# matvogel/P2P-Bridge

Hardware: AMD Instinct MI355X
Metric: denoised points/sec (8192-pt patches, T=30) (higher is better)
Workload: dtype f32; 1 GPU; PVDS_PUNet xyz-only, 8192-pt patches, T=30 bridge steps, batch 32 per GPU (BASELINE configs[1]); patches_per_gpu=32, points_per_patch=8192, bridge_steps=30, parallelism=patch-shard x1, process_group_world_size=1, hipgraph=True, weights=seeded random init (26.44 M params)

## Files before the change

### include/p2pb_hip.h

```cpp
#ifndef P2PB_HIP_H
#define P2PB_HIP_H

#include <stddef.h>

#ifdef __cplusplus
extern "C" {
#endif

#define P2PB_EINVAL (-22)

#define P2PB_ABI_VERSION 13

int p2pb_version(void);
const char *p2pb_target_arch(void);
int p2pb_set_split_terms(int terms);
int p2pb_set_split_terms_thread(int terms);
int p2pb_get_split_terms(void);
int p2pb_set_deterministic(int on);
int p2pb_get_deterministic(void);
int p2pb_debug_pointwise_form(int cin, int cout, int npos, unsigned long long *launches);

int p2pb_voxel_coords(int b, int n, int r, int normalize, float eps, const float *coords, float *norm,
                      int *vox, void *stream);

// ... 220 lines not shown
size_t p2pb_pointwise_minmax_floats(int b, int cout, int npos, int pool_u, int flags);
int p2pb_pointwise_conv_pool_forward(int b, int cin, int cout, int npos, const float *in, const void *wp,
                                     const float *bias, const float *bias_b, const float *in_scale,
                                     const float *in_shift, int in_swish, int flags, float *out, float *stats_part,
                                     int pool_u, float *minmax, double fin_count_per_channel, int fin_groups,
                                     const float *fin_gamma, const float *fin_beta, const float *fin_style, int fin_style_stride,
                                     float fin_eps, float *fin_scale, float *fin_shift, float *fin_chmean, void *stream);
int p2pb_pointwise_conv_pool_gather(int b, int cin, int cout, int n, int m, int u, const float *zt, const float *cxt,
                                    const int *idx, const void *wp_split, const float *bias, const float *in_scale,
                                    const float *in_shift, int in_swish, float *stats_part, float *minmax,
                                    double fin_count_per_channel, int fin_groups, const float *fin_gamma, const float *fin_beta,
                                    const float *fin_style, int fin_style_stride, float fin_eps, float *fin_scale,
                                    float *fin_shift, float *fin_chmean, void *stream);
int p2pb_linear_rows(int b, int cin, int cout, const float *x, long x_stride, const float *w, long w_stride,
                     const float *bias, float *out, long out_stride, void *stream);
int p2pb_minmax_act(int b, int c, int m, int nslots, const float *minmax, const float *scale, const float *shift,
                    int swish, float *y, void *stream);
int p2pb_minmax_act_pool_gn(int b, int c, int nslots, const float *minmax, const float *part, int nslots_st,
                            double count_per_channel, int groups, const float *gamma, const float *beta, const float *style,
                            int style_stride, float eps, int swish, float *scale, float *shift, float *y, void *stream);
int p2pb_affine_act(int b, int c, int npos, const float *x, const float *scale, const float *shift, int swish,
                    const float *residual, float *y, void *stream);
int p2pb_affine_act_max(int b, int c, int m, int u, const float *x, const float *scale, const float *shift,
                        int swish, float *y, void *stream);

int p2pb_linear_attention_forward(int b, int heads, int dim_head, int n, const float *qkv, float *out, float *ctx,
                                  void *stream);
int p2pb_linear_attention_backward(int b, int heads, int dim_head, int n, const float *qkv, const float *ctx,
                                   const float *grad_out, float *grad_qkv, void *stream);

// ... 154 lines not shown
```

### p2p_bridge_amd/_lib.py

```python
import ctypes
import os

import torch

_HERE = os.path.dirname(os.path.abspath(__file__))
LIB_PATH = os.environ.get("P2PB_LIB_PATH") or os.path.join(_HERE, "libp2pb_hip.so")

SYMBOLS = [
    "p2pb_version", "p2pb_target_arch", "p2pb_set_split_terms", "p2pb_set_split_terms_thread", "p2pb_get_split_terms", "p2pb_set_deterministic", "p2pb_get_deterministic", "p2pb_voxel_coords", "p2pb_avg_voxelize_ws_bytes",
    "p2pb_avg_voxelize_forward", "p2pb_avg_voxelize_backward", "p2pb_avg_voxelize_cl_gather_split", "p2pb_conv3d_presplit",
    "p2pb_conv3d_k3_forward_compact_pre", "p2pb_trilinear_devoxelize_forward",
    "p2pb_trilinear_devoxelize_backward", "p2pb_ball_query", "p2pb_grouping_forward", "p2pb_grouping_backward", "p2pb_group_concat", "p2pb_group_sub", "p2pb_three_interpolate_add", "p2pb_group_sub_stats_floats", "p2pb_group_sub_stats_slots", "p2pb_group_sub_stats",
    "p2pb_gather_features_forward", "p2pb_gather_features_backward", "p2pb_furthest_point_sampling",
    "p2pb_fps_coop_ws_bytes", "p2pb_furthest_point_sampling_coop", "p2pb_point_face_dist", "p2pb_face_point_dist", "p2pb_knn_points_ws_bytes", "p2pb_knn_points", "p2pb_three_nn_interpolate_forward", "p2pb_three_nn_interpolate_backward", "p2pb_three_nn", "p2pb_three_nn_cells", "p2pb_three_nn_cells_ws_bytes",
    "p2pb_three_interpolate", "p2pb_chamfer_forward",
    "p2pb_chamfer_backward", "p2pb_approxmatch_forward", "p2pb_matchcost_forward", "p2pb_matchcost_backward",
    "p2pb_auction_forward", "p2pb_auction_backward", "p2pb_conv3d_k3_packed_floats", "p2pb_conv3d_k3_pack_weights",
    "p2pb_conv3d_k3_split_packed_bytes", "p2pb_conv3d_k3_pack_weights_split",
    "p2pb_conv3d_k3_stats_floats", "p2pb_conv3d_k3_forward", "p2pb_conv3d_k3_forward_ex",
    "p2pb_conv3d_k3_far_field", "p2pb_conv3d_k3_far_field_gn", "p2pb_pvconv_tail", "p2pb_minmax_act_pool_gn", "p2pb_conv3d_active_lists", "p2pb_conv3d_k3_forward_compact", "p2pb_conv3d_brick_lists", "p2pb_conv3d_k3_forward_sparse", "p2pb_gn_affine_params", "p2pb_se_gate_affine",
    "p2pb_trilinear_devoxelize_affine", "p2pb_avg_voxelize_cl_forward", "p2pb_voxel_sort", "p2pb_avg_voxelize_cl_gather", "p2pb_trilinear_devoxelize_cl_affine", "p2pb_pointwise_packed_floats", "p2pb_pointwise_pack_weights",
    "p2pb_pointwise_stats_floats", "p2pb_pointwise_conv_forward", "p2pb_affine_act", "p2pb_affine_act_max",
    "p2pb_pointwise_split_packed_bytes", "p2pb_pointwise_pack_weights_split", "p2pb_pointwise_pool_supported", "p2pb_pointwise_minmax_floats", "p2pb_pointwise_conv_pool_forward",
    "p2pb_minmax_act", "p2pb_linear_attention_forward", "p2pb_linear_attention_backward", "p2pb_softmax_attention_forward", "p2pb_softmax_attention_backward",
    "p2pb_approxmatch_temp_floats", "p2pb_approxmatch_forward_ws", "p2pb_pointwise_conv_pool_gather", "p2pb_chamfer_ws_bytes", "p2pb_chamfer_forward_ws", "p2pb_radius_count", "p2pb_radius_fill", "p2pb_merge_accumulate", "p2pb_merge_finish", "p2pb_gn_affine_params_ex", "p2pb_norm_act_backward", "p2pb_norm_act_backward_ex", "p2pb_grouping_backward_pitched", "p2pb_three_nn_interpolate_backward_pitched", "p2pb_affine_act_train", "p2pb_conv3d_k3_wgrad_ws_floats", "p2pb_conv3d_k3_wgrad", "p2pb_conv3d_k3_wgrad_occ_ws_floats", "p2pb_conv3d_k3_wgrad_occ", "p2pb_pointwise_wgrad_ws_floats", "p2pb_pointwise_wgrad",
    "p2pb_debug_pointwise_form", "p2pb_linear_rows", "p2pb_fps_grid_ws_bytes", "p2pb_furthest_point_sampling_grid",
    "p2pb_optim_entry_bytes", "p2pb_optim_chunk", "p2pb_optim_clip_adam_step",
    "p2pb_conv3d_k3_pack_weights_split_adjoint", "p2pb_pointwise_pack_weights_adjoint", "p2pb_pointwise_pack_weights_split_adjoint",
    "p2pb_conv3d_k3_pack_weights_split_amax", "p2pb_pointwise_pack_weights_split_amax",
    "p2pb_se_gate_forward", "p2pb_se_gate_backward", "p2pb_row_max_forward", "p2pb_row_max_backward",
    "p2pb_pairwise_chamfer_ws_bytes", "p2pb_pairwise_chamfer", "p2pb_pairwise_emd_ws_bytes", "p2pb_pairwise_emd",
    "p2pb_occupancy_grid_cells", "p2pb_occupancy_ws_bytes", "p2pb_occupancy_counts",
    "p2pb_pn2_ball_query", "p2pb_pn2_three_nn", "p2pb_pn2_fps", "p2pb_pn2_three_interpolate", "p2pb_pn2_three_interpolate_grad",
    "p2pb_pointops_knnquery", "p2pb_pointops_ballquery", "p2pb_pointops_furthestsampling", "p2pb_pointops_grouping_forward",
    "p2pb_pointops_grouping_backward", "p2pb_pointops_interpolation_forward", "p2pb_pointops_interpolation_backward",
    "p2pb_pointops_subtraction_forward", "p2pb_pointops_subtraction_backward", "p2pb_pointops_aggregation_forward",
    "p2pb_pointops_aggregation_backward",
    "p2pb_imgfeat_visibility_ws_bytes", "p2pb_imgfeat_visibility", "p2pb_imgfeat_fuse", "p2pb_imgfeat_fill_round",
    "p2pb_scan_depth_valid", "p2pb_scan_backproject", "p2pb_scan_cell_keys", "p2pb_scan_segment_mean", "p2pb_scan_big_chunk_rows",
    "p2pb_scan_segment_mean_big", "p2pb_scan_radius_count", "p2pb_scan_knn_grid", "p2pb_scan_knn_brute",
    "p2pb_pairs_tri_areas", "p2pb_pairs_sample_mesh", "p2pb_pairs_knn", "p2pb_pairs_unique_assign", "p2pb_pairs_finish",
# ... 38 lines not shown
        _lib.p2pb_pointwise_minmax_floats.restype = ctypes.c_size_t
        _lib.p2pb_group_sub_stats_floats.restype = ctypes.c_size_t
        _lib.p2pb_pointwise_split_packed_bytes.restype = ctypes.c_size_t
        _lib.p2pb_conv3d_k3_wgrad_ws_floats.restype = ctypes.c_size_t
        _lib.p2pb_conv3d_k3_wgrad_occ_ws_floats.restype = ctypes.c_size_t
        _lib.p2pb_chamfer_ws_bytes.restype = ctypes.c_size_t
        _lib.p2pb_approxmatch_temp_floats.restype = ctypes.c_size_t
        _lib.p2pb_pointwise_wgrad_ws_floats.restype = ctypes.c_size_t
        _lib.p2pb_optim_entry_bytes.restype = ctypes.c_size_t
        _lib.p2pb_pairwise_chamfer_ws_bytes.restype = ctypes.c_size_t
        _lib.p2pb_pairwise_emd_ws_bytes.restype = ctypes.c_size_t
        _lib.p2pb_occupancy_ws_bytes.restype = ctypes.c_size_t
        _lib.p2pb_imgfeat_visibility_ws_bytes.restype = ctypes.c_size_t
        _lib.p2pb_vit_patch_embed_ws_floats.restype = ctypes.c_size_t
        _lib.p2pb_room_fps_jobs_ws_bytes.restype = ctypes.c_size_t
        have = _lib.p2pb_version() if hasattr(_lib, "p2pb_version") else None
        if have != ABI_VERSION:
            bad, _lib = _lib, None
            del bad
            raise P2PBError(f"{LIB_PATH} is ABI version {have}, this package binds version {ABI_VERSION} (include/p2pb_hip.h): "
                            "rebuild it with `python -m p2p_bridge_amd.build`")
        for s in SYMBOLS:
            getattr(_lib, s)
        _lib.p2pb_set_split_terms(6 if os.environ.get("P2PB_CONV_MATH") in ("bf16x6", "fp32") else 16)
    return _lib


def stream_ptr():
    return ctypes.c_void_p(torch.cuda.current_stream().cuda_stream)


# ... 18 lines not shown
```

### p2p_bridge_amd/csrc/pointwise_act.hip

```cpp
#include "pw_common.h"

__global__ __launch_bounds__(256) void minmax_act_kernel(int c, int m, int nslots, const float *__restrict__ mm,
                                                         const float *__restrict__ scale,
                                                         const float *__restrict__ shift, int swish,
                                                         float *__restrict__ y, size_t total) {
  for (size_t e = (size_t)blockIdx.x * 256 + threadIdx.x; e < total; e += (size_t)gridDim.x * 256) {
    float mn, mx;
    size_t bc;
    if (nslots == 0) {
      bc = e / m;
      const float2 v = *(const float2 *)(mm + e * 2);
      mn = v.x;
      mx = v.y;
    } else {
      bc = e;
      const size_t b = e / c, ch = e % c;
      mn = INFINITY;
      mx = -INFINITY;
      for (int sl = 0; sl < nslots; ++sl) {
        const float2 v = *(const float2 *)(mm + ((b * nslots + sl) * c + ch) * 2);
        mn = fminf(mn, v.x);
        mx = fmaxf(mx, v.y);
      }
    }
// ... 64 lines not shown
                                       double count_per_channel, int groups, const float *gamma, const float *beta,
                                       const float *style, int style_stride, float eps, int swish, float *scale, float *shift,
                                       float *y, void *stream) {
  if (b <= 0 || c <= 0 || nslots <= 0 || !minmax || !part || nslots_st <= 0 || !scale || !shift || !y || groups <= 0 ||
      c % groups != 0 || c / groups > 256 || (style && style_stride < 2 * c) || (size_t)c * 8 > 32 * 1024)
    return P2PB_EINVAL;
  GnFinish f = {};
  f.gamma = gamma, f.beta = beta, f.style = style, f.scale = scale, f.shift = shift, f.style_stride = style_stride, f.groups = groups;
  f.eps = eps, f.count_per_channel = count_per_channel;
  hipLaunchKernelGGL(minmax_act_pool_kernel, dim3((c + 31) / 32, b), dim3(256), (size_t)c * 8, (hipStream_t)stream, c, nslots, minmax,
                     (const float *)nullptr, (const float *)nullptr, swish, y, part, nslots_st, f);
  return p2pb_launch_status();
}

#define LR_BC 16
__global__ __launch_bounds__(256) void linear_rows_kernel(int B, int cin, int cout, const float *__restrict__ x, long xs,
                                                          const float *__restrict__ w, long ws,
                                                          const float *__restrict__ bias, float *__restrict__ out, long os,
                                                          int bc) {
  extern __shared__ float lr_x[];
  const int tid = threadIdx.x, lane = tid & 63, wave = tid >> 6, l31 = lane & 31, h = lane >> 5;
  const int row0 = blockIdx.x * 32;
  const int xp = cin + 4;
  const int wrow = min(row0 + l31, cout - 1);
  const int nk8 = (cin + 7) / 8;
  for (int b0 = 0; b0 < B; b0 += bc) {
    const int nb = min(bc, B - b0);
    __syncthreads();
    for (int e = tid * 4; e < nb * cin; e += 1024) {
      const int bb = e / cin, c = e - bb * cin;
      *(f32x4 *)(lr_x + bb * xp + c) = *(const f32x4 *)(x + (size_t)(b0 + bb) * xs + c);
    }
    __syncthreads();
    f32x16 acc;
// ... 20 lines not shown
      for (int u = 0; u < 8; ++u)
#pragma unroll
        for (int i = 0; i < 4; ++i) acc = __builtin_amdgcn_mfma_f32_32x32x2f32(wv[u][i], xv[u][i], acc, 0, 0, 0);
    }
    __syncthreads();
    float *red = lr_x;
    if (l31 < nb) {
#pragma unroll
      for (int r = 0; r < 16; ++r) red[(wave * 32 + (r & 3) + 8 * (r >> 2) + 4 * h) * 17 + l31] = acc[r];
    }
    __syncthreads();
    for (int e = tid; e < 32 * nb; e += 256) {
      const int r = e / nb, bb = e - r * nb;
      if (row0 + r < cout) {
        const float v = (red[(0 * 32 + r) * 17 + bb] + red[(1 * 32 + r) * 17 + bb]) + (red[(2 * 32 + r) * 17 + bb] + red[(3 * 32 + r) * 17 + bb]);
        out[(size_t)(b0 + bb) * os + row0 + r] = v + (bias ? bias[row0 + r] : 0.0f);
      }
    }
  }
}

extern "C" int p2pb_linear_rows(int b, int cin, int cout, const float *x, long x_stride, const float *w, long w_stride,
                                const float *bias, float *out, long out_stride, void *stream) {
  if (b <= 0 || cin <= 0 || cout <= 0 || !x || !w || !out || (cin & 3) || (x_stride & 3) || (w_stride & 3) ||
      (((uintptr_t)x | (uintptr_t)w) & 15) || x_stride < cin || w_stride < cin || out_stride < cout)
    return P2PB_EINVAL;
  int bc = (int)(65536 / ((long)(cin + 4) * 4));
  if (bc < 1) return P2PB_EINVAL;
  if (bc > LR_BC) bc = LR_BC;
  if (bc > b) bc = b;
  size_t lr_lds = (size_t)bc * (cin + 4) * 4;
  if (lr_lds < 4 * 32 * 17 * 4) lr_lds = 4 * 32 * 17 * 4;
  hipLaunchKernelGGL(linear_rows_kernel, dim3(cdiv(cout, 32)), dim3(256), lr_lds, (hipStream_t)stream, b, cin,
                     cout, x, x_stride, w, w_stride, bias, out, out_stride, bc);
  return p2pb_launch_status();
}

__global__ __launch_bounds__(256) void affine_act_kernel(int c, int P, const float *__restrict__ x,
                                                         const float *__restrict__ scale,
                                                         const float *__restrict__ shift, int swish,
                                                         const float *__restrict__ residual, float *__restrict__ y) {
  const int bc = blockIdx.y;
  const float sc = scale[bc], sh = shift[bc];
  const float *xr = x + (size_t)bc * P;
  const float *rr = residual ? residual + (size_t)bc * P : nullptr;
  float *yr = y + (size_t)bc * P;
  for (int p = blockIdx.x * 256 + threadIdx.x; p < P; p += gridDim.x * 256) {
    float v = xr[p] * sc + sh;
    if (swish) v = swishf(v);
// ... 98 lines not shown
```

### p2p_bridge_amd/fused.py

```python
import ctypes
import os

from . import _experiment
import threading

import torch

from ._lib import call, check, lib, ptr, stream_ptr

_i, _f, _d = ctypes.c_int, ctypes.c_float, ctypes.c_double
F32 = torch.float32


CONV_MATHS = ("f16x3", "bf16x6", "fp32")
SPLIT_MATHS = ("f16x3", "bf16x6")
CONV_MATH_DEFAULT = "f16x3"
_SPLIT_TERMS = {"f16x3": 16, "bf16x6": 6, "fp32": 6, "bf16x3": 3}
_conv_math_override = None


def conv_math() -> str:
    m = _conv_math_override or os.environ.get("P2PB_CONV_MATH", CONV_MATH_DEFAULT)
    if m not in CONV_MATHS:
        raise ValueError(f"P2PB_CONV_MATH must be one of {CONV_MATHS}, got {m!r}")
# ... 467 lines not shown

def linear_rows(x, weight, bias=None):
    if x.stride(-1) != 1 or x.data_ptr() % 16 or x.stride(0) % 4:
        x = x.contiguous()
    if weight.stride(-1) != 1 or weight.data_ptr() % 16 or weight.stride(0) % 4:
        weight = weight.contiguous()
    b, ci = x.shape
    co = weight.shape[0]
    assert weight.shape[1] == ci and x.dtype == F32 and weight.dtype == F32 and x.is_cuda
    out = torch.empty(b, co, dtype=F32, device=x.device)
    call("p2pb_linear_rows", _i(b), _i(ci), _i(co), ptr(x), ctypes.c_long(x.stride(0)), ptr(weight), ctypes.c_long(weight.stride(0)),
         ptr(bias), ptr(out), ctypes.c_long(co), stream_ptr())
    return out


def minmax_act(mm, scale, shift, swish=True, global_pool=False):
    if global_pool:
        b, nslots, c, _ = mm.shape
        y = torch.empty(b, c, dtype=F32, device=mm.device)
        m = 1
    else:
        b, c, m, _ = mm.shape
        nslots = 0
        y = torch.empty(b, c, m, dtype=F32, device=mm.device)
    call("p2pb_minmax_act", _i(b), _i(c), _i(m), _i(nslots), ptr(mm), ptr(scale), ptr(shift), _i(int(swish)), ptr(y),
         stream_ptr())
    return y


def gather_pool_supported(ci: int, co: int, m: int, u: int) -> bool:
# ... 132 lines not shown
```

### p2p_bridge_amd/p2pb.py

```python
import os
import warnings
from typing import Dict, List, Optional

import numpy as np
import torch
import torch.nn as nn

from .pvcnn_unet import PVCNN2Unet, _get


def space_indices(num_steps: int, count: int) -> List[int]:
    assert count <= num_steps
    stride = 1 if count <= 1 else (num_steps - 1) / (count - 1)
    cur, out = 0.0, []
    for _ in range(count):
        out.append(round(cur))
        cur += stride
    return out


def make_beta_schedule(n_timestep=1000, linear_start=1e-4, linear_end=2e-2):
    scale = 1000 / n_timestep
    a, b = (linear_start * scale) ** 0.5, (linear_end * scale) ** 0.5
    return (torch.linspace(a, b, n_timestep, dtype=torch.float64) ** 2).numpy()
# ... 232 lines not shown
        B = xt.shape[0]
        t = coef[0].expand(B)
        if self.cond_x1:
            x_cond = x1 if x_cond is None else torch.cat([x1, x_cond], dim=1)
        out = net(xt, t, x_cond=x_cond)
        if self.objective == "pred_noise":
            x0 = xt - coef[1] * out
            if clip:
                x0 = x0.clamp(-3.0, 3.0)
        else:
            x0 = out
        xt_prev = coef[2] * x0 + coef[3] * xt
        if noise is not None:
            xt_prev = xt_prev + coef[4] * noise
        return xt_prev, x0

    @torch.no_grad()
    def ddpm_sampling(self, x1, x_cond=None, clip_denoise=False, sampling_steps=None, log_count=10, verbose=True,
                      use_ema=False, graph=False):
        from . import fused

        args = (x1, x_cond, clip_denoise, sampling_steps, log_count, verbose, use_ema, graph)
        xs, x0s = self._ddpm_once(*args)
        policy = self.f16_overflow or os.environ.get("P2PB_F16_OVERFLOW", "rerun")
        if policy not in ("rerun", "raise", "ignore"):
            raise ValueError(f"P2PB_F16_OVERFLOW must be rerun | raise | ignore, got {policy!r}")
        if policy == "ignore" or fused.conv_math() != "f16x3" or xs.device.type != "cuda":
            return xs, x0s
        if bool(torch.isfinite(xs[:, 0]).all()):
            return xs, x0s
# ... 35 lines not shown
        if ema_was_training:
            self.ema.ema_model.eval()
        if self.add_x1_noise:
            x1 = x1 + torch.randn_like(x1)
        xt = x1.detach().to(self.device)
        xs, x0s = [], []
        rev = steps[::-1]
        chains = self._sampler_chains(xt) if graph else 1
        if chains > 1:
            try:
                return self._ddpm_chains(net, xt, x_cond, clip_denoise, rev, table, log_steps, chains)
            finally:
                if ema_was_training:
                    self.ema.ema_model.train()
                self.model.train()
        runner = self._graph_runner(net, xt, x_cond, clip_denoise) if graph else None
        try:
            for i, prev in enumerate(rev[1:]):
                noise = torch.randn_like(xt) if (not self.ot_ode and prev > 0) else None
                if runner is not None:
                    xt, x0 = runner(xt, table[i], noise)
                else:
                    xt, x0 = self._one_step(net, xt, table[i], x1, x_cond, clip_denoise, noise)
                if prev in log_steps:
                    xs.append(xt.clone() if runner is not None else xt)
                    x0s.append(x0.clone() if runner is not None else x0)
        finally:
            if ema_was_training:
                self.ema.ema_model.train()
            self.model.train()
        flip = lambda z: torch.flip(torch.stack(z, dim=1), dims=(1,))
        return flip(xs), flip(x0s)

    def _sampler_chains(self, xt) -> int:
        v = self.sample_chains if self.sample_chains is not None else os.environ.get("P2PB_SAMPLE_CHAINS")
        B, N = xt.shape[0], xt.shape[2]
        auto = 2 if (B % 2 == 0 and ((B >= 16 and N <= 16384) or (B >= 32 and N > 16384))) else 1
        k = int(v) if v not in (None, "", "auto") else auto
        return max(1, min(k, B))

    def _ddpm_chains(self, net, xt, x_cond, clip, rev, table, log_steps, chains):
        B = xt.shape[0]
        cuts = [(B * c) // chains for c in range(chains + 1)]
        parts = [slice(cuts[c], cuts[c + 1]) for c in range(chains)]
        main = torch.cuda.current_stream()
        runners = [self._graph_runner(net, xt[p], None if x_cond is None else x_cond[p], clip, chain=c)
                   for c, p in enumerate(parts)]
        streams = self._chain_streams = (getattr(self, "_chain_streams", None) or [])
        while len(streams) < chains:
            streams.append(torch.cuda.Stream(device=xt.device))
        if getattr(self, "_chains_serial", False):
            streams = [main] * chains
        x_c = [xt[p] for p in parts]
        logs = [([], []) for _ in parts]
        nsteps = len(rev) - 1
        for i, prev in enumerate(rev[1:]):
            noise = torch.randn_like(xt) if (not self.ot_ode and prev > 0) else None
            if noise is not None and i > 0:
                drawn = torch.cuda.Event()
                drawn.record(main)
                for c in range(chains):
                    streams[c].wait_event(drawn)
            if i == 0:
                from . import _experiment

                dflt = 0 if xt.shape[2] <= 16384 else 100
                phase = _experiment.get_int("chain_stagger_pct", dflt) / 100.0
                timed_first = phase > 0 and chains > 1 and nsteps > 1
                if timed_first:
                    e0, e1 = torch.cuda.Event(enable_timing=True), torch.cuda.Event(enable_timing=True)
                    e0.record(main)
                    x_c[0], x0 = runners[0](x_c[0], table[0], None if noise is None else noise[parts[0]])
                    e1.record(main)
                    if prev in log_steps:
                        logs[0][0].append(x_c[0].clone()), logs[0][1].append(x0.clone())
                    e1.synchronize()
                    step_ms = e0.elapsed_time(e1)
                for c in range(chains):
                    streams[c].wait_stream(main)
                    if timed_first and c > 0:
                        with torch.cuda.stream(streams[c]):
                            torch.cuda._sleep(int(step_ms * c / chains * phase * 1.8e6))
            for c in range(chains):
                if i == 0 and c == 0 and timed_first:
                    continue
                with torch.cuda.stream(streams[c]):
                    x_c[c], x0 = runners[c](x_c[c], table[i], None if noise is None else noise[parts[c]])
                    if prev in log_steps:
                        logs[c][0].append(x_c[c].clone()), logs[c][1].append(x0.clone())
                    if noise is not None:
                        noise.record_stream(streams[c])
        for c in range(chains):
            main.wait_stream(streams[c])
        flip = lambda z: torch.flip(torch.stack(z, dim=1), dims=(1,))
        xs = torch.cat([flip(l[0]) for l in logs], dim=0)
        x0s = torch.cat([flip(l[1]) for l in logs], dim=0)
        return xs, x0s

    @staticmethod
    def _weights_fingerprint(net):
        return tuple((t.data_ptr(), t._version) for t in list(net.parameters()) + list(net.buffers()))

    def _graph_runner(self, net, xt, x_cond, clip, chain=0):
        if self.cond_x1:
            raise NotImplementedError("graph capture with cond_x1")
        from . import fused

        key = (tuple(xt.shape), None if x_cond is None else tuple(x_cond.shape), bool(clip), id(net), fused.conv_math(), chain)
        fp = self._weights_fingerprint(net)
        entry = self._graphs.get(key)
        if entry is not None and entry[0] != fp:
            del self._graphs[key]
            entry = None
        if entry is None:
            s_x = xt.clone()
            s_c = torch.zeros(5, device=xt.device)
            s_n = None if self.ot_ode else torch.zeros_like(xt)
            s_cond = None if x_cond is None else x_cond.clone()
            self._one_step(net, s_x, s_c, None, s_cond, clip, s_n)
            torch.cuda.synchronize()
            side = torch.cuda.Stream()
            side.wait_stream(torch.cuda.current_stream())
            with torch.cuda.stream(side):
                for _ in range(2):
                    self._one_step(net, s_x, s_c, None, s_cond, clip, s_n)
            torch.cuda.current_stream().wait_stream(side)
            torch.cuda.synchronize()
            g = torch.cuda.CUDAGraph()
            with torch.cuda.graph(g, capture_error_mode="thread_local"):
                o_x, o_0 = self._one_step(net, s_x, s_c, None, s_cond, clip, s_n)
            entry = self._graphs[key] = (fp, g, s_x, s_c, s_n, s_cond, o_x, o_0)
        _, g, s_x, s_c, s_n, s_cond, o_x, o_0 = entry
        if s_cond is not None:
            s_cond.copy_(x_cond)

        def run(x, coef, noise=None):
            s_x.copy_(x)
            s_c.copy_(coef)
            if s_n is not None:
                if noise is None:
                    s_n.zero_()
                else:
                    s_n.copy_(noise)
            g.replay()
            return o_x, o_0

        return run

    @torch.no_grad()
    def calibrate_ranges(self, x_start, x_cond=None, steps=None, margin: float = 4.0, use_ema=False):
        from . import fused

        if fused.conv_math() != "f16x3" or self.device.type != "cuda":
            return []
        net = self.ema.ema_model if (use_ema and self.ema is not None) else self.model
        names = {id(m): n for n, m in net.named_modules()}
        was_training = net.training
        net.eval()
        _, table = self.step_tables(steps or self.timesteps - 1)
        xs = x_start.detach().to(self.device)
# ... 89 lines not shown
```

### p2p_bridge_amd/pvcnn_unet.py

```python
from dataclasses import dataclass
from typing import Any, List, Optional

import numpy as np
import os

import torch

from . import _experiment
import torch.nn as nn
import torch.nn.functional as F

from . import layers as L


def _get(cfg, key, default=None):
    if cfg is None:
        return default
    if isinstance(cfg, dict):
        v = cfg.get(key, None)
    else:
        v = getattr(cfg, key, None)
        if v is None and hasattr(cfg, "get"):
            v = cfg.get(key, None)
    return default if v is None else v


@dataclass
class PVCData:
    features: torch.Tensor
    coords: torch.Tensor = None
    cond_coords: torch.Tensor = None
    cond_features: torch.Tensor = None
    lower_coords: torch.Tensor = None
    lower_features: torch.Tensor = None
    time_emb: torch.Tensor = None
    cond: Any = None
    geo: Any = None
    lower_temb: torch.Tensor = None


def temb_broadcast(base, m):
    out = base[:, :, None].expand(-1, -1, m)
    out._p2pb_base = base
    return out


def temb_at(time_emb, m):
    base = getattr(time_emb, "_p2pb_base", None)
    if base is not None:
        return temb_broadcast(base, m)
    return time_emb[:, :, :m] if m <= time_emb.shape[-1] else time_emb[:, :, 0:1].expand(-1, -1, m)


# ... 602 lines not shown
        self.mlp = SharedMLP(in_channels, list(out_channels), dim=1, gn_groups=gn_groups, cond_dim=cond_dim)

    def forward(self, data: PVCData) -> PVCData:
        if data.geo is not None:
            idx, w = data.geo.take_fp(self.level)
            from . import fused

            if fused.enabled(self.mlp, data.lower_features):
                conv0 = self.mlp.layers[0]
                g = data.lower_features.contiguous()
                cg = g.shape[1]
                pm = g.shape[2] % 4 == 0
                tb = None
                if data.lower_temb is not None:
                    e = data.lower_temb.shape[1]
                    tb = fused.linear_rows(data.lower_temb, conv0.weight.reshape(conv0.weight.shape[0], -1)[:, cg:cg + e])
                cz, _ = fused.pw_conv(g, conv0, stats=False, ci_lo=0, ci_hi=cg, use_bias=False, point_major=pm, bias_b=tb)
                if tb is not None:
                    cg += data.lower_temb.shape[1]
                skip = data.features
                if skip is not None:
                    ys, _ = fused.pw_conv(skip.contiguous(), conv0, stats=False, ci_lo=cg, ci_hi=cg + skip.shape[1])
                    y, st = fused.interp_add(cz, idx, w, add=ys, point_major=pm)
                else:
                    y, st = fused.interp_add(cz, idx, w, bias=conv0.bias, point_major=pm)
                if data.time_emb is not None:
                    data.time_emb = data.time_emb[:, :, 0:1].expand(-1, -1, data.coords.shape[-1])
                data.features = self.mlp._run_fused(y, data.cond, False, None, first=st)
                return data
            x = L.three_interpolate(data.lower_features.contiguous(), idx, w)
        else:
# ... 121 lines not shown
        sa.append(dict(convs=convs, centers=ncen, radius=radius[i], neighbors=32, mlp_in=mlp_in, mlp_out=mlp_out))
        cin = mlp_out[-1]
    sa_in[0] = feat_dim + input_dim
    fp_mlps = [[channels[3], channels[3]], [channels[3], channels[3]], [channels[3], channels[2]],
               [channels[2], channels[2], channels[1]]]
    fp_conv = [(channels[3], n_fp_blocks[3], voxel_resolutions[3]), (channels[3], n_fp_blocks[2], voxel_resolutions[2]),
               (channels[2], n_fp_blocks[1], voxel_resolutions[1]), (channels[1], n_fp_blocks[0], voxel_resolutions[0])]
    fp = []
    for j in range(4):
        mlp_in = cin + sa_in[-1 - j] + embed_dim
        convs = []
        c = fp_mlps[j][-1]
        for _ in range(fp_conv[j][1]):
            convs.append(dict(cin=c, cout=fp_conv[j][0], r=int(fp_conv[j][2])))
            c = fp_conv[j][0]
        fp.append(dict(mlp_in=mlp_in, mlp_out=fp_mlps[j], convs=convs))
        cin = c
    return dict(sa=sa, fp=fp, bottleneck=sa[-1]["mlp_out"][-1], out=cin)


class Geometry:

    def __init__(self, plan, coords, side):
        main = torch.cuda.current_stream()
        self.main = main
        c0 = coords.contiguous()
        side.wait_stream(main)
        self.sa, self.fp = [], []
        from . import fused

        self.voxel = {}
# ... 162 lines not shown
        self._dec_adagn = None
        self._pass = {"drop_seed": None}
        for k, m in enumerate(m for m in self.modules() if isinstance(m, PVConv)):
            m._pass, m.drop_salt = self._pass, k + 1

    def get_timestep_embedding(self, timesteps, device=None):
        if timesteps.dim() == 2 and timesteps.shape[1] == 1:
            timesteps = timesteps[:, 0]
        assert timesteps.dim() == 1, f"get shape: {timesteps.shape}"
        e = timesteps[:, None] * self._temb_freq[None, :]
        e = torch.cat([torch.sin(e), torch.cos(e)], dim=1)
        if self.embed_dim % 2 == 1:
            e = F.pad(e, (0, 1), "constant", 0)
        return e

    def _decoder_adagns(self):
        if self._dec_adagn is None:
            self._dec_adagn = {id(m) for part in (self.global_att, self.fp_layers, self.classifier) if part is not None
                               for m in part.modules() if isinstance(m, AdaGN)}
        return self._dec_adagn

    def forward(self, x, t, x_cond=None):
        if x_cond is not None:
            x = torch.cat([x, x_cond], dim=1)
        B, C, N = x.shape
        assert C == self.input_dim + self.extra_feature_channels, \
            f"input dim: {C}, expected: {self.input_dim + self.extra_feature_channels}"
        coords = x[:, : self.input_dim].contiguous()
        feats = x[:, self.input_dim:].contiguous()
        from . import fused
# ... 29 lines not shown
            from . import dense

            if dense.fold_step_neighbours():
                self._pass["drop_seed"] = dense.dropout_seed(x.device)
        time_emb = None
        if t is not None:
            if t.dim() == 0:
                t = t.view(1).expand(B)
            te = self.get_timestep_embedding(t)
            if use_fused:
                te = fused.linear_rows(te, self.embedf[0].weight, self.embedf[0].bias)
                te = fused.linear_rows(F.leaky_relu(te, self.embedf[1].negative_slope), self.embedf[2].weight, self.embedf[2].bias)
            else:
                te = self.embedf(te)
            time_emb = temb_broadcast(te, N)
        data = PVCData(features=feats, coords=coords, time_emb=time_emb, cond=cond, geo=geo)

        skips, level_coords = [feats], []
        for i, stage in enumerate(self.sa_layers):
            if i > 0:
                skips.append(data.features)
            level_coords.append(data.coords)
            if i > 0 and data.time_emb is not None:
                data.features = torch.cat([data.features, data.time_emb], dim=1)
            data = stage(data)

        if self.collect_cut and torch.is_grad_enabled():
            def alias(x):
                return x.view_as(x) if x.requires_grad else x

# ... 8 lines not shown
                cut += cond.cut
            self.cut = [x for x in cut if x.requires_grad]

        if self.global_att is not None:
            data.features = self.global_att(data.features)

        for j, stage in enumerate(self.fp_layers):
            ltemb = None
            if data.time_emb is None:
                lower = data.features
            elif use_fused and geo is not None and data.time_emb.shape[1] % 4 == 0 and data.features.shape[1] % 4 == 0:
                lower, ltemb = data.features, data.time_emb[:, :, 0]
            else:
                lower = torch.cat([data.features, data.time_emb], dim=1)
            data = stage(PVCData(features=skips[-1 - j], coords=level_coords[-1 - j], lower_coords=data.coords,
                                 lower_features=lower, time_emb=data.time_emb, cond=data.cond, geo=geo, lower_temb=ltemb))
        if geo is not None:
            geo.finish()

        if use_fused:
            c0 = self.classifier[0]
            xin = data.features.contiguous()
            h, st, (sc, sh, _) = fused.pw_conv(xin, c0.layers[0], fin=norm_fin(c0.layers[1], xin.shape[2], None))
            return fused.pw_conv(h, self.classifier[2], sc, sh, swish=True, stats=False)[0]
        from . import dense

        seed = self._pass["drop_seed"]
        if seed is not None:
            h = self.classifier[0].run(data.features, None, dropout=(float(self.classifier[1].p), seed, 0))
        else:
            h = self.classifier[1](self.classifier[0].run(data.features, None))
# ... 2 lines not shown
```

Baseline: 1.230 million points/s.

## Fuse bridge update and step advance into captured graph; batch FP time biases

The per-step bridge update (x0 estimate, clamp, next xt with noise) becomes a single vectorized kernel captured inside the HIP graph. A device-side advance kernel reads the coefficient row from a table, so the host no longer copies coefficients or xt before each replay. The per-FP-stage time-embedding bias linears are also merged into one segmented linear launch at the start of the forward. Together these remove several small elementwise launches and host copies per step, at the cost of device-side step state that must be reset correctly for every sampling call.

```diff
diff --git a/include/p2pb_hip.h b/include/p2pb_hip.h
--- a/include/p2pb_hip.h
+++ b/include/p2pb_hip.h
@@ -258,6 +258,11 @@
                                     float *fin_shift, float *fin_chmean, void *stream);
 int p2pb_linear_rows(int b, int cin, int cout, const float *x, long x_stride, const float *w, long w_stride,
                      const float *bias, float *out, long out_stride, void *stream);
+int p2pb_linear_rows_segments(int b, int cin, int nseg, const int *seg_start, const float *x, long x_stride, const float *w,
+                              long w_stride, const float *bias, float *out, void *stream);
+int p2pb_bridge_step(long n, int pred_noise, int clamp, const float *xt, const float *out, const float *coef,
+                     const float *noise, float *x0, float *xt_prev, void *stream);
+int p2pb_bridge_advance(int reset, int nsteps, int cap, const float *table, int *state, float *coef, void *stream);
 int p2pb_minmax_act(int b, int c, int m, int nslots, const float *minmax, const float *scale, const float *shift,
                     int swish, float *y, void *stream);
 int p2pb_minmax_act_pool_gn(int b, int c, int nslots, const float *minmax, const float *part, int nslots_st,
diff --git a/p2p_bridge_amd/_lib.py b/p2p_bridge_amd/_lib.py
--- a/p2p_bridge_amd/_lib.py
+++ b/p2p_bridge_amd/_lib.py
@@ -24,7 +24,7 @@
     "p2pb_pointwise_split_packed_bytes", "p2pb_pointwise_pack_weights_split", "p2pb_pointwise_pool_supported", "p2pb_pointwise_minmax_floats", "p2pb_pointwise_conv_pool_forward",
     "p2pb_minmax_act", "p2pb_linear_attention_forward", "p2pb_linear_attention_backward", "p2pb_softmax_attention_forward", "p2pb_softmax_attention_backward",
     "p2pb_approxmatch_temp_floats", "p2pb_approxmatch_forward_ws", "p2pb_pointwise_conv_pool_gather", "p2pb_chamfer_ws_bytes", "p2pb_chamfer_forward_ws", "p2pb_radius_count", "p2pb_radius_fill", "p2pb_merge_accumulate", "p2pb_merge_finish", "p2pb_gn_affine_params_ex", "p2pb_norm_act_backward", "p2pb_norm_act_backward_ex", "p2pb_grouping_backward_pitched", "p2pb_three_nn_interpolate_backward_pitched", "p2pb_affine_act_train", "p2pb_conv3d_k3_wgrad_ws_floats", "p2pb_conv3d_k3_wgrad", "p2pb_conv3d_k3_wgrad_occ_ws_floats", "p2pb_conv3d_k3_wgrad_occ", "p2pb_pointwise_wgrad_ws_floats", "p2pb_pointwise_wgrad",
-    "p2pb_debug_pointwise_form", "p2pb_linear_rows", "p2pb_fps_grid_ws_bytes", "p2pb_furthest_point_sampling_grid",
+    "p2pb_debug_pointwise_form", "p2pb_linear_rows", "p2pb_bridge_step", "p2pb_bridge_advance", "p2pb_linear_rows_segments", "p2pb_fps_grid_ws_bytes", "p2pb_furthest_point_sampling_grid",
     "p2pb_optim_entry_bytes", "p2pb_optim_chunk", "p2pb_optim_clip_adam_step",
     "p2pb_conv3d_k3_pack_weights_split_adjoint", "p2pb_pointwise_pack_weights_adjoint", "p2pb_pointwise_pack_weights_split_adjoint",
     "p2pb_conv3d_k3_pack_weights_split_amax", "p2pb_pointwise_pack_weights_split_amax",
@@ -93,7 +93,7 @@
         _lib.p2pb_imgfeat_visibility_ws_bytes.restype = ctypes.c_size_t
         _lib.p2pb_vit_patch_embed_ws_floats.restype = ctypes.c_size_t
         _lib.p2pb_room_fps_jobs_ws_bytes.restype = ctypes.c_size_t
-        have = _lib.p2pb_version() if hasattr(_lib, "p2pb_version") else None
+        have =_lib.p2pb_version() if hasattr(_lib, "p2pb_version") else None
         if have != ABI_VERSION:
             bad, _lib = _lib, None
             del bad
diff --git a/p2p_bridge_amd/csrc/bridge_step.hip b/p2p_bridge_amd/csrc/bridge_step.hip
--- /dev/null
+++ b/p2p_bridge_amd/csrc/bridge_step.hip
@@ -0,0 +1,100 @@
+#include "common.h"
+
+typedef float bs_f4 __attribute__((ext_vector_type(4)));
+
+template <bool PRED_NOISE, bool CLAMP, bool NOISE>
+__device__ __forceinline__ void bridge_one(float xt, float out, float nz, float c1, float c2, float c3, float c4, float &x0,
+                                           float &xp) {
+  float v = out;
+  if (PRED_NOISE) {
+    v = __fsub_rn(xt, __fmul_rn(c1, out));
+    if (CLAMP) v = (v != v) ? v : fminf(fmaxf(v, -3.0f), 3.0f);
+  }
+  float p = __fadd_rn(__fmul_rn(c2, v), __fmul_rn(c3, xt));
+  if (NOISE) p = __fadd_rn(p, __fmul_rn(c4, nz));
+  x0 = v;
+  xp = p;
+}
+
+template <bool PRED_NOISE, bool CLAMP, bool NOISE>
+__global__ __launch_bounds__(256) void bridge_step_kernel(size_t n, size_t nvec, const float *xt, const float *__restrict__ out,
+                                                          const float *__restrict__ coef, const float *__restrict__ noise,
+                                                          float *__restrict__ x0, float *xt_prev) {
+  const size_t i = (size_t)blockIdx.x * 256 + threadIdx.x;
+  const float c1 = coef[1], c2 = coef[2], c3 = coef[3], c4 = coef[4];
+  if (i < nvec) {
+    const bs_f4 a = ((const bs_f4 *)xt)[i], o = ((const bs_f4 *)out)[i];
+    bs_f4 z = {0.0f, 0.0f, 0.0f, 0.0f};
+    if (NOISE) z = ((const bs_f4 *)noise)[i];
+    bs_f4 v, p;
+#pragma unroll
+    for (int k = 0; k < 4; ++k) {
+      float vk, pk;
+      bridge_one<PRED_NOISE, CLAMP, NOISE>(a[k], o[k], z[k], c1, c2, c3, c4, vk, pk);
+      v[k] = vk;
+      p[k] = pk;
+    }
+    ((bs_f4 *)x0)[i] = v;
+    ((bs_f4 *)xt_prev)[i] = p;
+    return;
+  }
+  const size_t e = 4 * nvec + (i - nvec);
+  if (e >= n) return;
+  float vk, pk;
+  bridge_one<PRED_NOISE, CLAMP, NOISE>(xt[e], out[e], NOISE ? noise[e] : 0.0f, c1, c2, c3, c4, vk, pk);
+  x0[e] = vk;
+  xt_prev[e] = pk;
+}
+
+template <bool PRED_NOISE, bool CLAMP>
+static void bridge_launch(size_t n, size_t nvec, const float *xt, const float *out, const float *coef, const float *noise, float *x0,
+                          float *xt_prev, hipStream_t s) {
+  const size_t threads = nvec + (n - 4 * nvec);
+  const dim3 grid((unsigned)((threads + 255) / 256));
+  if (noise)
+    hipLaunchKernelGGL((bridge_step_kernel<PRED_NOISE, CLAMP, true>), grid, dim3(256), 0, s, n, nvec, xt, out, coef, noise, x0,
+                       xt_prev);
+  else
+    hipLaunchKernelGGL((bridge_step_kernel<PRED_NOISE, CLAMP, false>), grid, dim3(256), 0, s, n, nvec, xt, out, coef, noise, x0,
+                       xt_prev);
+}
+
+extern "C" int p2pb_bridge_step(long n, int pred_noise, int clamp, const float *xt, const float *out, const float *coef,
+                                const float *noise, float *x0, float *xt_prev, void *stream) {
+  if (n <= 0 || !xt || !out || !coef || !x0 || !xt_prev) return P2PB_EINVAL;
+  if (n > ((long)1 << 40)) return P2PB_EINVAL;
+  if (x0 == xt || x0 == out || x0 == xt_prev) return P2PB_EINVAL;
+  const size_t align = (size_t)xt | (size_t)out | (size_t)noise | (size_t)x0 | (size_t)xt_prev;
+  const size_t nvec = (align & 15) == 0 ? (size_t)n / 4 : 0;
+  hipStream_t s = (hipStream_t)stream;
+  if (!pred_noise)
+    bridge_launch<false, false>((size_t)n, nvec, xt, out, coef, noise, x0, xt_prev, s);
+  else if (clamp)
+    bridge_launch<true, true>((size_t)n, nvec, xt, out, coef, noise, x0, xt_prev, s);
+  else
+    bridge_launch<true, false>((size_t)n, nvec, xt, out, coef, noise, x0, xt_prev, s);
+  return p2pb_launch_status();
+}
+
+__global__ void bridge_advance_kernel(int reset, int nsteps, int cap, const float *__restrict__ table, int *__restrict__ state,
+                                      float *__restrict__ coef) {
+  if (threadIdx.x != 0 || blockIdx.x != 0) return;
+  int k = 0;
+  if (reset) {
+    state[0] = 0;
+    state[1] = nsteps;
+  } else {
+    k = state[0] + 1;
+    nsteps = state[1];
+    state[0] = k;
+  }
+  if (k < 0 || k >= nsteps || k >= cap) return;
+  for (int j = 0; j < 5; ++j) coef[j] = table[(size_t)k * 5 + j];
+}
+
+extern "C" int p2pb_bridge_advance(int reset, int nsteps, int cap, const float *table, int *state, float *coef, void *stream) {
+  if (!table || !state || !coef || cap <= 0) return P2PB_EINVAL;
+  if (reset && (nsteps <= 0 || nsteps > cap)) return P2PB_EINVAL;
+  hipLaunchKernelGGL(bridge_advance_kernel, dim3(1), dim3(64), 0, (hipStream_t)stream, reset, nsteps, cap, table, state, coef);
+  return p2pb_launch_status();
+}
diff --git a/p2p_bridge_amd/csrc/pointwise_act.hip b/p2p_bridge_amd/csrc/pointwise_act.hip
--- a/p2p_bridge_amd/csrc/pointwise_act.hip
+++ b/p2p_bridge_amd/csrc/pointwise_act.hip
@@ -102,10 +102,16 @@
 }
 
 #define LR_BC 16
+#define LR_MAX_SEG 8
+struct LrSegs {
+  int n;
+  int start[LR_MAX_SEG + 1];
+};
+template <bool SEG>
 __global__ __launch_bounds__(256) void linear_rows_kernel(int B, int cin, int cout, const float *__restrict__ x, long xs,
                                                           const float *__restrict__ w, long ws,
                                                           const float *__restrict__ bias, float *__restrict__ out, long os,
-                                                          int bc) {
+                                                          int bc, LrSegs segs) {
   extern __shared__ float lr_x[];
   const int tid = threadIdx.x, lane = tid & 63, wave = tid >> 6, l31 = lane & 31, h = lane >> 5;
   const int row0 = blockIdx.x * 32;
@@ -156,7 +162,13 @@
       const int r = e / nb, bb = e - r * nb;
       if (row0 + r < cout) {
         const float v = (red[(0 * 32 + r) * 17 + bb] + red[(1 * 32 + r) * 17 + bb]) + (red[(2 * 32 + r) * 17 + bb] + red[(3 * 32 + r) * 17 + bb]);
-        out[(size_t)(b0 + bb) * os + row0 + r] = v + (bias ? bias[row0 + r] : 0.0f);
+        size_t o = (size_t)(b0 + bb) * os + row0 + r;
+        if (SEG) {
+          int j = 0;
+          while (j + 1 < segs.n && row0 + r >= segs.start[j + 1]) ++j;
+          o = (size_t)B * segs.start[j] + (size_t)(b0 + bb) * (segs.start[j + 1] - segs.start[j]) + (row0 + r - segs.start[j]);
+        }
+        out[o] = v + (bias ? bias[row0 + r] : 0.0f);
       }
     }
   }
@@ -173,8 +185,31 @@
   if (bc > b) bc = b;
   size_t lr_lds = (size_t)bc * (cin + 4) * 4;
   if (lr_lds < 4 * 32 * 17 * 4) lr_lds = 4 * 32 * 17 * 4;
-  hipLaunchKernelGGL(linear_rows_kernel, dim3(cdiv(cout, 32)), dim3(256), lr_lds, (hipStream_t)stream, b, cin,
-                     cout, x, x_stride, w, w_stride, bias, out, out_stride, bc);
+  hipLaunchKernelGGL(linear_rows_kernel<false>, dim3(cdiv(cout, 32)), dim3(256), lr_lds, (hipStream_t)stream, b, cin,
+                     cout, x, x_stride, w, w_stride, bias, out, out_stride, bc, LrSegs{});
+  return p2pb_launch_status();
+}
+
+extern "C" int p2pb_linear_rows_segments(int b, int cin, int nseg, const int *seg_start, const float *x, long x_stride,
+                                         const float *w, long w_stride, const float *bias, float *out, void *stream) {
+  if (nseg <= 0 || nseg > LR_MAX_SEG || !seg_start || seg_start[0] != 0) return P2PB_EINVAL;
+  LrSegs segs;
+  segs.n = nseg;
+  for (int j = 0; j <= LR_MAX_SEG; ++j) segs.start[j] = seg_start[j < nseg ? j : nseg];
+  for (int j = 0; j < nseg; ++j)
+    if (seg_start[j + 1] <= seg_start[j]) return P2PB_EINVAL;
+  const int cout = seg_start[nseg];
+  if (b <= 0 || cin <= 0 || !x || !w || !out || (cin & 3) || (x_stride & 3) || (w_stride & 3) ||
+      (((uintptr_t)x | (uintptr_t)w) & 15) || x_stride < cin || w_stride < cin)
+    return P2PB_EINVAL;
+  int bc = (int)(65536 / ((long)(cin + 4) * 4));
+  if (bc < 1) return P2PB_EINVAL;
+  if (bc > LR_BC) bc = LR_BC;
+  if (bc > b) bc = b;
+  size_t lr_lds = (size_t)bc * (cin + 4) * 4;
+  if (lr_lds < 4 * 32 * 17 * 4) lr_lds = 4 * 32 * 17 * 4;
+  hipLaunchKernelGGL(linear_rows_kernel<true>, dim3(cdiv(cout, 32)), dim3(256), lr_lds, (hipStream_t)stream, b, cin, cout, x,
+                     x_stride, w, w_stride, bias, out, (long)cout, bc, segs);
   return p2pb_launch_status();
 }
 
diff --git a/p2p_bridge_amd/fused.py b/p2p_bridge_amd/fused.py
--- a/p2p_bridge_amd/fused.py
+++ b/p2p_bridge_amd/fused.py
@@ -505,6 +505,43 @@
     return out
 
 
+def linear_rows_segments(x, weight, sizes, bias=None):
+    if x.stride(-1) != 1 or x.data_ptr() % 16 or x.stride(0) % 4:
+        x = x.contiguous()
+    check(weight, F32, "weight")
+    b, ci = x.shape
+    co = weight.shape[0]
+    assert weight.shape[1] == ci and x.dtype == F32 and x.is_cuda and sum(sizes) == co and 0 < len(sizes) <= 8
+    starts = [0]
+    for s in sizes:
+        starts.append(starts[-1] + int(s))
+    out = torch.empty(b * co, dtype=F32, device=x.device)
+    call("p2pb_linear_rows_segments", _i(b), _i(ci), _i(len(sizes)), (ctypes.c_int * len(starts))(*starts), ptr(x),
+         ctypes.c_long(x.stride(0)), ptr(weight), ctypes.c_long(weight.stride(0)), ptr(bias), ptr(out), stream_ptr())
+    return [out[b * lo:b * hi].view(b, hi - lo) for lo, hi in zip(starts[:-1], starts[1:])]
+
+
+def bridge_step(xt, out, coef, noise=None, pred_noise=True, clip=False, x0=None, xt_prev=None):
+    for t, name in ((xt, "xt"), (out, "out"), (coef, "coef")) + (() if noise is None else ((noise, "noise"),)):
+        check(t, F32, name)
+    assert out.shape == xt.shape and coef.numel() >= 5 and (noise is None or noise.shape == xt.shape)
+    x0 = torch.empty_like(xt) if x0 is None else x0
+    xt_prev = torch.empty_like(xt) if xt_prev is None else xt_prev
+    for t, name in ((x0, "x0"), (xt_prev, "xt_prev")):
+        check(t, F32, name)
+        assert t.shape == xt.shape
+    call("p2pb_bridge_step", ctypes.c_long(xt.numel()), _i(bool(pred_noise)), _i(bool(clip)), ptr(xt), ptr(out), ptr(coef),
+         ptr(noise), ptr(x0), ptr(xt_prev), stream_ptr())
+    return xt_prev, x0
+
+
+def bridge_advance(table, state, coef, reset_steps=None):
+    check(table, F32, "table"), check(coef, F32, "coef"), check(state, torch.int32, "state")
+    assert table.dim() == 2 and table.shape[1] == 5 and state.numel() >= 2 and coef.numel() >= 5
+    call("p2pb_bridge_advance", _i(reset_steps is not None), _i(reset_steps or 0), _i(table.shape[0]), ptr(table), ptr(state),
+         ptr(coef), stream_ptr())
+
+
 def minmax_act(mm, scale, shift, swish=True, global_pool=False):
     if global_pool:
         b, nslots, c, _ = mm.shape
diff --git a/p2p_bridge_amd/p2pb.py b/p2p_bridge_amd/p2pb.py
--- a/p2p_bridge_amd/p2pb.py
+++ b/p2p_bridge_amd/p2pb.py
@@ -270,6 +270,15 @@
         if noise is not None:
             xt_prev = xt_prev + coef[4] * noise
         return xt_prev, x0
+
+    def _captured_step(self, net, s_x, s_c, s_cond, clip, s_n, o_0, s_tab, s_k):
+        from . import fused
+
+        out = net(s_x, s_c[0].expand(s_x.shape[0]), x_cond=s_cond)
+        if not out.is_contiguous():
+            out = out.contiguous()
+        fused.bridge_step(s_x, out, s_c, s_n, pred_noise=self.objective == "pred_noise", clip=clip, x0=o_0, xt_prev=s_x)
+        fused.bridge_advance(s_tab, s_k, s_c)
 
     @torch.no_grad()
     def ddpm_sampling(self, x1, x_cond=None, clip_denoise=False, sampling_steps=None, log_count=10, verbose=True,
@@ -335,12 +344,12 @@
                 if ema_was_training:
                     self.ema.ema_model.train()
                 self.model.train()
-        runner = self._graph_runner(net, xt, x_cond, clip_denoise) if graph else None
+        runner = self._graph_runner(net, xt, x_cond, clip_denoise, table) if graph else None
         try:
             for i, prev in enumerate(rev[1:]):
                 noise = torch.randn_like(xt) if (not self.ot_ode and prev > 0) else None
                 if runner is not None:
-                    xt, x0 = runner(xt, table[i], noise)
+                    xt, x0 = runner(xt, noise)
                 else:
                     xt, x0 = self._one_step(net, xt, table[i], x1, x_cond, clip_denoise, noise)
                 if prev in log_steps:
@@ -365,7 +374,7 @@
         cuts = [(B * c) // chains for c in range(chains + 1)]
         parts = [slice(cuts[c], cuts[c + 1]) for c in range(chains)]
         main = torch.cuda.current_stream()
-        runners = [self._graph_runner(net, xt[p], None if x_cond is None else x_cond[p], clip, chain=c)
+        runners = [self._graph_runner(net, xt[p], None if x_cond is None else x_cond[p], clip, table, chain=c)
                    for c, p in enumerate(parts)]
         streams = self._chain_streams = (getattr(self, "_chain_streams", None) or [])
         while len(streams) < chains:
@@ -391,7 +400,7 @@
                 if timed_first:
                     e0, e1 = torch.cuda.Event(enable_timing=True), torch.cuda.Event(enable_timing=True)
                     e0.record(main)
-                    x_c[0], x0 = runners[0](x_c[0], table[0], None if noise is None else noise[parts[0]])
+                    x_c[0], x0 = runners[0](x_c[0], None if noise is None else noise[parts[0]])
                     e1.record(main)
                     if prev in log_steps:
                         logs[0][0].append(x_c[0].clone()), logs[0][1].append(x0.clone())
@@ -406,7 +415,7 @@
                 if i == 0 and c == 0 and timed_first:
                     continue
                 with torch.cuda.stream(streams[c]):
-                    x_c[c], x0 = runners[c](x_c[c], table[i], None if noise is None else noise[parts[c]])
+                    x_c[c], x0 = runners[c](x_c[c], None if noise is None else noise[parts[c]])
                     if prev in log_steps:
                         logs[c][0].append(x_c[c].clone()), logs[c][1].append(x0.clone())
                     if noise is not None:
@@ -422,7 +431,7 @@
     def _weights_fingerprint(net):
         return tuple((t.data_ptr(), t._version) for t in list(net.parameters()) + list(net.buffers()))
 
-    def _graph_runner(self, net, xt, x_cond, clip, chain=0):
+    def _graph_runner(self, net, xt, x_cond, clip, table, chain=0):
         if self.cond_x1:
             raise NotImplementedError("graph capture with cond_x1")
         from . import fused
@@ -438,33 +447,41 @@
             s_c = torch.zeros(5, device=xt.device)
             s_n = None if self.ot_ode else torch.zeros_like(xt)
             s_cond = None if x_cond is None else x_cond.clone()
-            self._one_step(net, s_x, s_c, None, s_cond, clip, s_n)
+            o_0 = torch.empty_like(xt)
+            s_tab = torch.zeros(self.timesteps, 5, device=xt.device)
+            s_k = torch.zeros(2, dtype=torch.int32, device=xt.device)
+            step = lambda: self._captured_step(net, s_x, s_c, s_cond, clip, s_n, o_0, s_tab, s_k)
+            step()
             torch.cuda.synchronize()
             side = torch.cuda.Stream()
             side.wait_stream(torch.cuda.current_stream())
             with torch.cuda.stream(side):
                 for _ in range(2):
-                    self._one_step(net, s_x, s_c, None, s_cond, clip, s_n)
+                    s_x.copy_(xt)
+                    step()
             torch.cuda.current_stream().wait_stream(side)
             torch.cuda.synchronize()
             g = torch.cuda.CUDAGraph()
             with torch.cuda.graph(g, capture_error_mode="thread_local"):
-                o_x, o_0 = self._one_step(net, s_x, s_c, None, s_cond, clip, s_n)
-            entry = self._graphs[key] = (fp, g, s_x, s_c, s_n, s_cond, o_x, o_0)
-        _, g, s_x, s_c, s_n, s_cond, o_x, o_0 = entry
+                step()
+            entry = self._graphs[key] = (fp, g, s_x, s_c, s_n, s_cond, o_0, s_tab, s_k)
+        _, g, s_x, s_c, s_n, s_cond, o_0, s_tab, s_k = entry
         if s_cond is not None:
             s_cond.copy_(x_cond)
-
-        def run(x, coef, noise=None):
-            s_x.copy_(x)
-            s_c.copy_(coef)
+        assert table.shape[0] <= s_tab.shape[0]
+        s_tab[: table.shape[0]].copy_(table)
+        fused.bridge_advance(s_tab, s_k, s_c, reset_steps=table.shape[0])
+
+        def run(x, noise=None):
+            if x is not s_x:
+                s_x.copy_(x)
             if s_n is not None:
                 if noise is None:
                     s_n.zero_()
                 else:
                     s_n.copy_(noise)
             g.replay()
-            return o_x, o_0
+            return s_x, o_0
 
         return run
 
diff --git a/p2p_bridge_amd/pvcnn_unet.py b/p2p_bridge_amd/pvcnn_unet.py
--- a/p2p_bridge_amd/pvcnn_unet.py
+++ b/p2p_bridge_amd/pvcnn_unet.py
@@ -37,6 +37,7 @@
     cond: Any = None
     geo: Any = None
     lower_temb: torch.Tensor = None
+    lower_tbias: torch.Tensor = None
 
 
 def temb_broadcast(base, m):
@@ -669,7 +670,9 @@
                 tb = None
                 if data.lower_temb is not None:
                     e = data.lower_temb.shape[1]
-                    tb = fused.linear_rows(data.lower_temb, conv0.weight.reshape(conv0.weight.shape[0], -1)[:, cg:cg + e])
+                    tb = data.lower_tbias
+                    if tb is None:
+                        tb = fused.linear_rows(data.lower_temb, conv0.weight.reshape(conv0.weight.shape[0], -1)[:, cg:cg + e])
                 cz, _ = fused.pw_conv(g, conv0, stats=False, ci_lo=0, ci_hi=cg, use_bias=False, point_major=pm, bias_b=tb)
                 if tb is not None:
                     cg += data.lower_temb.shape[1]
@@ -821,7 +824,7 @@
         for _ in range(fp_conv[j][1]):
             convs.append(dict(cin=c, cout=fp_conv[j][0], r=int(fp_conv[j][2])))
             c = fp_conv[j][0]
-        fp.append(dict(mlp_in=mlp_in, mlp_out=fp_mlps[j], convs=convs))
+        fp.append(dict(mlp_in=mlp_in, mlp_out=fp_mlps[j], convs=convs, lower=cin))
         cin = c
     return dict(sa=sa, fp=fp, bottleneck=sa[-1]["mlp_out"][-1], out=cin)
 
@@ -1014,6 +1017,23 @@
             e = F.pad(e, (0, 1), "constant", 0)
         return e
 
+    def _fp_time_biases(self, te):
+        from . import _experiment, fused
+
+        e = te.shape[1]
+        if e % 4 or _experiment.get_int("fp_tbias", 1) == 0:
+            return None
+        convs = [(s[0] if isinstance(s, _Stage) else s).mlp.layers[0] for s in self.fp_layers]
+        if len(convs) > 8 or any(st["lower"] % 4 for st in self.plan["fp"]):
+            return None
+        key = tuple((c.weight.data_ptr(), c.weight._version) for c in convs)
+        if getattr(self, "_fp_tbias_pack", (None,))[0] != key:
+            cols = [c.weight.detach().reshape(c.weight.shape[0], -1)[:, st["lower"]:st["lower"] + e]
+                    for c, st in zip(convs, self.plan["fp"])]
+            self._fp_tbias_pack = (key, torch.cat(cols, dim=0).contiguous(), [c.shape[0] for c in cols])
+        _, w, sizes = self._fp_tbias_pack
+        return fused.linear_rows_segments(te, w, sizes)
+
     def _decoder_adagns(self):
         if self._dec_adagn is None:
             self._dec_adagn = {id(m) for part in (self.global_att, self.fp_layers, self.classifier) if part is not None
@@ -1073,6 +1093,7 @@
             else:
                 te = self.embedf(te)
             time_emb = temb_broadcast(te, N)
+        fp_tbias = self._fp_time_biases(te) if (time_emb is not None and use_fused and geo is not None) else None
         data = PVCData(features=feats, coords=coords, time_emb=time_emb, cond=cond, geo=geo)
 
         skips, level_coords = [feats], []
@@ -1111,7 +1132,9 @@
             else:
                 lower = torch.cat([data.features, data.time_emb], dim=1)
             data = stage(PVCData(features=skips[-1 - j], coords=level_coords[-1 - j], lower_coords=data.coords,
-                                 lower_features=lower, time_emb=data.time_emb, cond=data.cond, geo=geo, lower_temb=ltemb))
+                                 lower_features=lower, time_emb=data.time_emb, cond=data.cond, geo=geo, lower_temb=ltemb,
+                                 lower_tbias=fp_tbias[j] if (ltemb is not None and fp_tbias is not None
+                                                             and lower.shape[1] == self.plan["fp"][j]["lower"]) else None))
         if geo is not None:
             geo.finish()
 
```

New measurement: 1.237 million points/s, median of 6. No clear change (+0.6%).
